# tomer196/GaUDI

Hardware: AMD Instinct MI355X
Metric: guided molecules/sec (1000-step) (higher is better)
Workload: dtype f32

## Files before the change

gaudi_amd/csrc/gaudi_hip.hip:

```cpp
#include <hip/hip_runtime.h>

#include <algorithm>
#include <climits>
#include <queue>
#include <cmath>
#include <cstdio>
#include <cstdlib>
#include <chrono>
#include <cstring>
#include <map>
#include <mutex>
#include <string>
#include <vector>

#include "../../include/gaudi_hip.h"
#include "kernel_table.h"

using namespace gaudi;

struct DevBuf {
  void* p = nullptr;
  size_t cap = 0;
  hipError_t reserve(size_t bytes) {
    if (bytes <= cap) return hipSuccess;
// ... 80 lines not shown
  struct VtCall {
    const gaudi_target_spec* spec = nullptr;
    int K = 0, Btot = 0, b0 = 0;
    float* trace = nullptr;
  }* vt = nullptr;
  PinBuf p_pred, p_dpred;
  PinBuf p_z, p_dz;
  DevBuf d_dz;
  hipEvent_t cb_event = nullptr;
  int steps_per_launch = 25;
  int variant = 8;
  LaunchPlan plan;
  bool split = true;
  bool no_fr = false;
  bool no_n1 = false;
  std::string last_key;
  std::vector<std::string> key_log;
  bool wide_full = true;
  bool gn8_pq = true;
  bool gn8 = true;
  bool force_gn8 = false;
  bool pack = true;
  int pairs_cap = -1;
  int pairs = 1;
  int num_cus = 256;
  bool pred_rounds = true;
  bool pack_now = false;
  bool force_mr = false;
  bool force_gn = false;
  bool fix_noise = false;
// ... 537 lines not shown
      for (int k = 0; k < ns; ++k)
        if (sl[k].live && sl[k].j == j) idx[n_out++] = (uint16_t)k;
    }
    off[N] = (uint16_t)n_out;
  }
  M.order.resize(B);
  for (int b = 0; b < B; ++b) M.order[b] = b;
  std::stable_sort(M.order.begin(), M.order.end(), [&](int a, int c) {
    return M.ntiles[a] != M.ntiles[c] ? M.ntiles[a] > M.ntiles[c] : total[a] > total[c];
  });
  return GAUDI_OK;
}

KernelTable* gaudi::g_kernel_tables;

static kernel_fn find_kernel(const KernelKey& k) {
  for (const KernelTable* t = g_kernel_tables; t; t = t->next)
    for (int i = 0; i < t->n; ++i)
      if (t->entries[i].key == k) return t->entries[i].fn;
  return nullptr;
}
static std::string key_name(const KernelKey& k) {
  char buf[160];
  snprintf(buf, sizeof buf, "waves=%d SP=%d MR=%d GN=%d FR=%d PG=%d N1=%d EF=%d HPE=%d HPP=%d VT=%d", k.waves, k.sp, (int)k.mr, k.gn,
           (int)k.fr, (int)k.pg, (int)k.n1, k.ef, k.hpe, k.hpp, (int)k.vt);
  return buf;
}
static std::string duplicate_kernel_key() {
  std::vector<KernelKey> seen;
  for (const KernelTable* t = g_kernel_tables; t; t = t->next)
    for (int i = 0; i < t->n; ++i) {
      if (std::find(seen.begin(), seen.end(), t->entries[i].key) != seen.end()) return key_name(t->entries[i].key);
      seen.push_back(t->entries[i].key);
    }
  return "";
// ... 172 lines not shown
    }
  }
#else
  if (h->prof) {
    KParams PC = P;
    HIPCHECK(h, h->d_clock.reserve(sizeof(unsigned long long) * 4));
    PC.clock_out = h->d_clock.as<unsigned long long>();
    hipLaunchKernelGGL(fn, dim3(P.B), dim3(v8 ? w8::kThreads : kThreads), lds, h->stream, PC);
  } else {
    hipLaunchKernelGGL(fn, dim3(P.B), dim3(v8 ? w8::kThreads : kThreads), lds, h->stream, P);
  }
#endif
  HIPCHECK(h, hipGetLastError());
  h->last_key = key_name(key);
  if (std::find(h->key_log.begin(), h->key_log.end(), h->last_key) == h->key_log.end()) h->key_log.push_back(h->last_key);
  if (h->prof) {
    HIPCHECK(h, h->prof_log.end(h->stream, ev));
    h->prof_steps += steps;
  }
  return GAUDI_OK;
}

struct Pack {
  int G = 0;
  int NG = 0;
  std::vector<float> umask, uemask;
  std::vector<uint8_t> align;
  std::vector<int32_t> rowmap;
  std::vector<int32_t> compmol;
  std::vector<int32_t> ncomp;
// ... 264 lines not shown
  P.NR = N;
  P.EW = M.S;
  P.node_mask = h->d_mask.as<float>();
  P.order = h->d_order.as<int>();
  P.edges = h->d_edges.as<uint32_t>();
  P.emask = h->d_emask.as<float>();
  P.npairs = h->d_npairs.as<int>();
  P.seginfo = h->d_seg.as<uint32_t>();
  P.ncols = h->d_ncols.as<int>();
  P.soff = h->d_soff.as<uint16_t>();
  P.sidx = h->d_sidx.as<uint16_t>();
  P.rowmap = packed ? h->d_rowmap.as<int32_t>() : nullptr;
  P.compmol = packed ? h->d_compmol.as<int32_t>() : nullptr;
  P.ncomp = packed ? h->d_ncomp.as<int32_t>() : nullptr;
  P.hk_off = 0;
  int hk = 0;
  if (h->keep_h && GAUDI_NODE_F16 && acc.mode >= 1 && nodes == kResident) {
    const size_t floats = lds_bytes8(hpe, hpp, n_slots, Dz, M.S, acc.pubx, acc.mode) / sizeof(float);
    const size_t at = (floats + 3) & ~(size_t)3;
    const size_t need = (size_t)w8::nh_keep_floats(std::max(hpe, hpp), n_slots);
    if ((at + need) * sizeof(float) + 1024 <= 160 * 1024) {
      P.hk_off = (int)at;
      hk = (int)need;
    }
  }
  if (pg_run) {
    const size_t stride = ((size_t)n_slots * (hpp + 4) + 63) / 64 * 64;
    HIPCHECK(h, h->d_gnode.reserve(sizeof(float) * (stride * (size_t)B + 256)));
    P.gnode = h->d_gnode.as<float>();
    P.gnode_stride = (long long)stride;
  }
  if (gn8) {
    const size_t stride = (gnode_floats8(hpe, hpp, N) + 63) / 64 * 64;
    HIPCHECK(h, h->d_gnode.reserve(sizeof(float) * (stride * (size_t)B + 256)));
    P.gnode = h->d_gnode.as<float>();
    P.gnode_stride = (long long)stride;
  }
  plan.waves = 8;
  plan.ring = acc.mode;
  plan.mr = mr_run;
// ... 122 lines not shown
  if (const char* v = getenv("GAUDI_PACK")) h->pack = atoi(v) != 0;
  if (const char* v = getenv("GAUDI_GN8_PACK")) h->gn8_pack = atoi(v) != 0;
  if (const char* v = getenv("GAUDI_GN8_PQ")) h->gn8_pq = atoi(v) != 0;
  if (const char* v = getenv("GAUDI_WIDE_FULL")) h->wide_full = atoi(v) != 0;
  if (const char* v = getenv("GAUDI_KEEP_H")) h->keep_h = atoi(v) != 0;
  if (const char* v = getenv("GAUDI_FAMILY_SPLIT")) h->family_split = atoi(v) != 0;
  if (const char* v = getenv("GAUDI_PAIRS")) h->pairs = atoi(v);
  if (const char* v = getenv("GAUDI_PAIRS_CAP")) h->pairs_cap = atoi(v);
  {
    int cus = 0;
    if (hipDeviceGetAttribute(&cus, hipDeviceAttributeMultiprocessorCount, device) == hipSuccess && cus > 0) h->num_cus = cus;
  }
  if (const char* v = getenv("GAUDI_PRED_ROUNDS")) h->pred_rounds = atoi(v) != 0;
  h->no_fr = getenv("GAUDI_NO_FR") != nullptr;
  h->no_n1 = getenv("GAUDI_NO_N1") != nullptr;
  h->plan.waves = h->variant;
  if (hipSetDevice(device) != hipSuccess || hipStreamCreateWithFlags(&h->stream, hipStreamNonBlocking) != hipSuccess) {
    delete h;
    return GAUDI_E_HIP;
  }
  *out = h;
  return GAUDI_OK;
}

void gaudi_destroy(gaudi_handle* h) {
  if (!h) return;
  (void)hipSetDevice(h->device);
  if (h->stream) (void)hipStreamSynchronize(h->stream);
  h->prof_log.reset(true);
  h->stab_log.reset(true);
// ... 1373 lines not shown
```

gaudi_amd/csrc/kern8s1_fused_192_208.hip:

```cpp
#include "kernel_table.h"

namespace {
using namespace gaudi;
using V = V8T<1, false, 0, false, false, true>;
const KernelEntry kEntries[] = {
    entry<V, 192, 208>(),
};
KernelTable kTable(kEntries);
}
```

gaudi_amd/csrc/kernel_table.h:

```cpp
#pragma once
#include "sampler_kernel.h"

namespace gaudi {

typedef void (*kernel_fn)(const KParams);

struct KernelKey {
  int waves;
  int sp;
  bool mr;
  int gn;
  bool fr, pg;
  bool n1;
  int ef;
  int hpe, hpp;
  bool vt;
};
inline bool operator==(const KernelKey& a, const KernelKey& b) {
  return a.waves == b.waves && a.sp == b.sp && a.mr == b.mr && a.gn == b.gn && a.fr == b.fr && a.pg == b.pg && a.n1 == b.n1 && a.ef == b.ef &&
         a.hpe == b.hpe && a.hpp == b.hpp && a.vt == b.vt;
}

struct KernelEntry {
  KernelKey key;
  kernel_fn fn;
};
template <class V, int HPE, int HPP, bool VT = false>
constexpr KernelEntry entry() {
  KernelEntry e{};
  e.key.waves = V::kWaveCount;
  e.key.sp = V::kSplit;
  e.key.mr = V::kMR;
  e.key.gn = V::kGN;
  e.key.fr = V::kFR;
  e.key.pg = V::kPG;
  e.key.n1 = V::kN1;
  e.key.ef = V::kEF;
  e.key.hpe = HPE;
  e.key.hpp = HPP;
  e.key.vt = VT;
  e.fn = &sampler_kernel_v<V, HPE, HPP, VT>;
  return e;
}

struct KernelTable {
  const KernelEntry* entries;
  int n;
  KernelTable* next;
  template <int N>
  explicit KernelTable(const KernelEntry (&e)[N]);
};
extern KernelTable* g_kernel_tables;
template <int N>
KernelTable::KernelTable(const KernelEntry (&e)[N]) : entries(e), n(N), next(g_kernel_tables) {
  g_kernel_tables = this;
}
// ... 3 lines not shown
```

gaudi_amd/csrc/sampler_kernel.h:

```cpp
#pragma once
#include "edm_device.h"
#include "pred_device.h"
#include "w8_edm.h"
#include "w8_pred.h"

#ifndef GAUDI_STATIC_PRIO
#define GAUDI_STATIC_PRIO 0
#endif

namespace gaudi {

enum Mode { MODE_PHI = 0, MODE_SAMPLE = 1, MODE_PRED_FWD = 2, MODE_PRED_GRAD = 3, MODE_GUIDE = 4, MODE_NLL = 5 };

struct KParams {
  int mode, B, N, F, EW;
  int NR;
  int do_init, do_decode, guided;
  int s_hi, s_lo, T;
  const float* node_mask;
  const int* order;
  const uint32_t* edges;
  const float* emask;
  const int* npairs;
  const uint32_t* seginfo;
// ... 28 lines not shown
  float* stash;
  long long stash_stride;
  float readout_div;
  const float* alpha_sigma;
  float* zt_out;
  int split;
  float* chain_out;
  int keep_frames;
  unsigned long long* stamps;
  float* gnode;
  long long gnode_stride;
  const int32_t* rowmap;
  const int32_t* compmol;
  const int32_t* ncomp;
  unsigned long long* clock_out;
  int hk_off;
  const struct VtDev* vt;
};
struct VtDev {
  const float* par;
  float* trace;
  int top;
  int B;
};
__device__ __forceinline__ const float* vt_row(const VtDev* vt, int b, int K) { return vt->par + (size_t)b * target_row_floats(K); }
__device__ __forceinline__ float* vt_trace_row(const VtDev* vt, int b, int K, int srow) {
  float* const t = vt->trace;
  return t != nullptr ? t + ((size_t)(vt->top - srow) * vt->B + b) * (K + 2) : nullptr;
}
constexpr int kMaxComp = 4;
// ... 1 lines not shown
__host__ __device__ inline int common_floats(int N, int D, int EW) {
  return 3 * align16(N * D) + align16(N) + 16 + align16(N) + 16 + 2 * kWaves * EW + align16(N);
}
__host__ __device__ inline int common_floats8(int N, int D, int S) {
  return 3 * align16(N * D) + align16(N) + 16 + align16(N) + 16 + 2 * S + align16(N) + align16((N + 1 + S + 1) / 2);
}
__device__ __forceinline__ int row_of(int w) { return w & 0x0fffffff; }
__device__ __forceinline__ int comp_of(int w) { return (w >> 28) & 7; }

template <bool GN, int EF = 2>
struct V4T {
  static constexpr int kThreads = gaudi::kThreads;
  static constexpr bool kGlobalNodes = GN;
  static constexpr int kWaveCount = 4, kSplit = 0, kGN = GN ? 1 : 0, kEF = EF;
  static constexpr bool kMR = false, kFR = false, kPG = false, kN1 = false;
  using Graph = gaudi::MolGraph;
  template <int HP> using EdmSmem = gaudi::NetSmem<HP, GN, EF>;
  __device__ __forceinline__ static void set_rows(Graph&, const int*, int, int) {}
  __host__ __device__ static int graph_floats(int N, int EW) { return 2 * gaudi::kWaves * EW + align16(N); }
  __device__ __forceinline__ static float* load_graph(const KParams& P, int b, float* base, const float* sMask, Graph& mg, int tid, int wave) {
    const int N = P.N, EW = P.EW;
    uint32_t* sEdge = (uint32_t*)base; base += gaudi::kWaves * EW;
    float* sEm = base; base += gaudi::kWaves * EW;
    uint32_t* sSeg = (uint32_t*)base; base += align16(N);
    for (int i = tid; i < N; i += kThreads) sSeg[i] = P.seginfo[b * N + i];
    for (int i = tid; i < gaudi::kWaves * EW; i += kThreads) {
      sEdge[i] = P.edges[(size_t)b * gaudi::kWaves * EW + i];
      sEm[i] = P.emask[(size_t)b * gaudi::kWaves * EW + i];
    }
    mg.N = N; mg.D = 3 + P.F; mg.EW = EW;
// ... 134 lines not shown
}
#ifndef GAUDI_STAMPS
template <int HP, int SP, int GN = 0, int FL = 0>
__device__ __attribute__((noinline)) void edm8_call(EdmDev W_, Graph8Args ga_, float t_val_, float* gnode_ = nullptr) {
  extern __shared__ __attribute__((aligned(16))) float smem[];
  const EdmDev W = uni(W_);
  const Graph8Args ga = uni(ga_);
  const float t_val = uni(t_val_);
  const Lds8 L = carve_lds8(smem, ga.N, ga.D, ga.S);
  const w8::MolGraph mg = graph8(L, ga);
  w8::NetSmem<HP, SP, GN> sm;
  sm.carve(L.net, ga.N, ga.S, GN ? uni(gnode_) : nullptr);
  sm.hk = ga.hk ? smem + ga.hk : nullptr;
  w8::edm_forward<HP, SP, GN, FL>(W, mg, sm, L.sZ, L.sEps, L.sMean, t_val, (int)threadIdx.x);
}
template <int HP, int SP, bool MR, int GN = 0, int FL = 0, bool PG = false>
__device__ __attribute__((noinline)) void pred_fwd8_call(PredDev W_, Graph8Args ga_, float t_val_, float* stash_, float readout_div_,
                                                         float* gnode_ = nullptr) {
  extern __shared__ __attribute__((aligned(16))) float smem[];
  const PredDev W = uni(W_);
  const Graph8Args ga = uni(ga_);
  const Lds8 L = carve_lds8(smem, ga.N, ga.D, ga.S);
  const w8::MolGraph mg = graph8(L, ga);
  w8::PredSmem<HP, SP, GN, PG> sm;
  sm.carve(L.net, ga.N, ga.S, ga.pubx, (GN || PG) ? uni(gnode_) : nullptr);
  sm.hk = ga.hk ? smem + ga.hk : nullptr;
  w8::pred_forward<HP, SP, MR, GN, FL>(W, mg, sm, L.sZ, uni(t_val_), uni(stash_), uni(readout_div_), (int)threadIdx.x);
}
template <int HP, int SP, bool MR, int GN = 0, int FL = 0, bool PG = false>
__device__ __attribute__((noinline)) void pred_bwd8_call(PredDev W_, Graph8Args ga_, float* stash_, float readout_div_, int resume_,
                                                         float* gnode_ = nullptr) {
  extern __shared__ __attribute__((aligned(16))) float smem[];
  const PredDev W = uni(W_);
  const Graph8Args ga = uni(ga_);
  const Lds8 L = carve_lds8(smem, ga.N, ga.D, ga.S);
  const w8::MolGraph mg = graph8(L, ga);
  w8::PredSmem<HP, SP, GN, PG> sm;
  sm.carve(L.net, ga.N, ga.S, ga.pubx, (GN || PG) ? uni(gnode_) : nullptr);
  w8::pred_backward<HP, SP, MR, GN, FL>(W, mg, sm, uni(stash_), L.sEps , uni(readout_div_), ga.pub_ch, (int)threadIdx.x,
                        uni(resume_) ? L.sZ : nullptr);
}
#endif

template <int SP, bool MR = false, int GN = 0, bool FR = false, bool PG = false, bool N1 = false>
struct V8T {
  static_assert(!N1 || (!MR && GN == 0 && !FR && !PG), "N1 is a form of the plain resident kernel");
  static constexpr int kFL = N1 ? w8::kNodeOneTile : (MR || GN != 0 || FR) ? w8::kNodeFresh : w8::kNodePlain;
  static constexpr int kThreads = w8::kThreads;
  static constexpr int kSplit = SP;
  static constexpr int kWaveCount = 8, kGN = GN, kEF = 2;
  static constexpr bool kMR = MR, kFR = FR, kPG = PG, kN1 = N1;
  using Graph = w8::MolGraph;
  __host__ __device__ static int graph_floats(int N, int S) { return 2 * S + align16(N) + align16((N + 1 + S + 1) / 2); }
  __device__ __forceinline__ static float* load_graph(const KParams& P, int b, float* base, const float* sMask, Graph& mg, int tid, int wave) {
    (void)wave;
    const int N = P.N, S = P.EW;
    uint32_t* sEdge = (uint32_t*)base; base += S;
    float* sEm = base; base += S;
    uint32_t* sSeg = (uint32_t*)base; base += align16(N);
    uint16_t* sOff = (uint16_t*)base;
    uint16_t* sIdx = sOff + (N + 1);
    base += align16((N + 1 + S + 1) / 2);
    for (int i = tid; i < N; i += kThreads) sSeg[i] = P.seginfo[b * N + i];
    for (int i = tid; i < N + 1; i += kThreads) sOff[i] = P.soff[(size_t)b * (N + 1) + i];
    for (int i = tid; i < S; i += kThreads) {
      sEdge[i] = P.edges[(size_t)b * S + i];
      sEm[i] = P.emask[(size_t)b * S + i];
      sIdx[i] = P.sidx[(size_t)b * S + i];
    }
    mg.N = N; mg.D = 3 + P.F; mg.S = S;
    mg.NC = P.ncols[b];
    mg.ntiles = P.npairs[b];
    mg.rounds = (mg.ntiles + w8::kWaves - 1) / w8::kWaves;
    mg.pubx = P.pubx;
    mg.pub_ch = P.pub_ch;
    mg.hk = P.hk_off;
    mg.mask = sMask; mg.edge = sEdge; mg.em = sEm; mg.seg = sSeg; mg.soff = sOff; mg.sidx = sIdx;
    return base;
  }
  __device__ __forceinline__ static void set_rows(Graph& mg, const int* row, int ncomp, int NR) { mg.row = row; mg.ncomp = ncomp; mg.NR = NR; }
  __device__ __forceinline__ static Graph8Args gargs(const Graph& mg) {
    return Graph8Args{mg.N, mg.D, mg.S, mg.NC, mg.ntiles, mg.pubx, mg.pub_ch, mg.hk};
  }
  static constexpr bool kGlobalNodes = GN != 0 || PG;
  template <int HP>
  __device__ __forceinline__ static void edm(const EdmDev& W, const Graph& mg, float* net, const float* sZ, float* sEps,
                                             float* sMean, float t_val, int tid STAMP_DECL, float* gnode) {
#ifdef GAUDI_STAMPS
    w8::NetSmem<HP, SP, GN> sm;
    sm.carve(net, mg.N, mg.S, GN ? uni(gnode) : nullptr);
    sm.hk = w8::lds_at(mg.hk);
// ... 6 lines not shown
  template <int HP>
  __device__ __forceinline__ static void guide(const PredDev& W, const Graph& mg, float* net, float* sZ, float* sGrad, float* sTmp,
                                               float* sMean, float t_val, float sigma, const float* target_w, float scale,
                                               float* pred_out, float readout_div, float* stash, int tid STAMP_DECL, int phase,
                                               const float* dpred_ext, float* gnode, const float* dz_ext, const VtDev* vt,
                                               int b, int srow) {
#ifdef GAUDI_STAMPS
    (void)vt; (void)b; (void)srow;
    (void)dz_ext;
    w8::guidance_update<HP, SP, MR, GN, PG>(W, mg, net, sZ, sGrad, sTmp, sMean, t_val, sigma, target_w, scale, pred_out, readout_div, stash,
                                            mg.pubx, mg.pub_ch, tid STAMP_ARGS, phase, dpred_ext, (GN || PG) ? uni(gnode) : nullptr);
#else
    (void)sTmp;
    w8::PredSmem<HP, SP, GN, PG> sm;
    sm.carve(net, mg.N, mg.S, mg.pubx, gnode);
    if (phase != 2) pred_fwd8_call<HP, SP, MR, GN, kFL, PG>(W, gargs(mg), t_val, stash, readout_div, gnode);
    if (vt != nullptr) vt_seed8(vt, b, srow, W.K, (int)(sm.pred - lds_base()));
    else w8::guidance_seed(W, sm, target_w, scale, pred_out, tid, phase, dpred_ext);
    if (phase == 1) return;
    pred_bwd8_call<HP, SP, MR, GN, kFL, PG>(W, gargs(mg), stash, readout_div, phase == 2 ? 1 : 0, gnode);
    if (dz_ext != nullptr) {
      for (int e = tid; e < mg.N * mg.D; e += kThreads) sGrad[e] += dz_ext[e];
      __syncthreads();
    }
    if (vt != nullptr) vt_norm8(vt, b, srow, W.K, mg.N * mg.D, (int)(sGrad - lds_base()));
    w8::guidance_apply(mg, sZ, sGrad, sMean, sigma, tid);
    if (vt != nullptr) vt_clip8(vt, b, srow, W.K, (int)(sMean - lds_base()));
#endif
  }
  template <int HP>
  __device__ __forceinline__ static void pred_entry(const PredDev& W, const Graph& mg, float* net, float* sZ, float* sGrad,
// ... 373 lines not shown
```

gaudi_amd/csrc/w8_common.h:

```cpp
#pragma once
#include <type_traits>

#include "device_common.h"

namespace gaudi {
namespace w8 {

constexpr int kWaves = 8;
constexpr int kThreads = 512;

template <int SH>
__device__ __forceinline__ float row_shr(float v) {
  return __builtin_bit_cast(float, __builtin_amdgcn_update_dpp(0, __builtin_bit_cast(int, v), 0x110 + SH, 0xF, 0xF, true));
}

template <int N, class F>
__device__ __forceinline__ void static_for_n(F f) {
  if constexpr (N > 0) {
    static_for_n<N - 1>(f);
    f(std::integral_constant<int, N - 1>{});
  }
}

struct RunMask {
// ... 451 lines not shown
  for (int u = wave; u < units; u += kWaves)
    __builtin_amdgcn_global_load_lds((const __attribute__((address_space(1))) void*)(g + u * 256 + lane * 4),
                                     (__attribute__((address_space(3))) void*)(lds + u * 256), 16, 0, 0);
}
__device__ __forceinline__ void stage_wait() {
  asm volatile("s_waitcnt vmcnt(0)" ::: "memory");
  __syncthreads();
}
__host__ __device__ __forceinline__ constexpr int stage_stride(int floats) { return (floats + 255) & ~255; }

struct MolGraph {
  int N, D, S;
  int NC;
  int ntiles, rounds;
  int pubx, pub_ch;
  int hk = 0;
  const float* mask;
  const uint32_t* edge;
  const float* em;
  const uint32_t* seg;
  const uint16_t* soff;
  const uint16_t* sidx;
  const int* row;
  int ncomp;
  int NR;
};
__device__ __forceinline__ float* lds_at(int off) {
  extern __shared__ __attribute__((aligned(16))) float gaudi_lds_alias[];
  return off ? gaudi_lds_alias + off : nullptr;
}
// ... 5 lines not shown
```

gaudi_amd/csrc/w8_nodes_f16.h:

```cpp
#pragma once
#include "w8_split.h"

namespace gaudi {
namespace w8 {


constexpr float kLoScale = 2048.f;
#ifndef GAUDI_NODE_ABLATE
#define GAUDI_NODE_ABLATE 0
#endif
constexpr int kAblateH = GAUDI_NODE_ABLATE;
#ifndef GAUDI_NODE_STAMPS
#define GAUDI_NODE_STAMPS 0
#endif
#ifndef GAUDI_NODE_PRIO
#define GAUDI_NODE_PRIO 1
#endif
struct NodeStampH {
  unsigned long long sum[8], last;
  __device__ __forceinline__ void start() { last = __builtin_amdgcn_s_memtime(); }
  __device__ __forceinline__ void mark(int i) {
    const unsigned long long t = __builtin_amdgcn_s_memtime();
    sum[i] += t - last;
    last = t;
// ... 178 lines not shown
constexpr int kNodePlain = 0;
constexpr int kNodeFresh = 1;
constexpr int kNodeOneTile = 2;
constexpr int kTailRuntime = 0;
constexpr int kTailOne = 1;

struct NodeCtxH {
  float winv;
  float* split_a;
  float* split_b;
  bool ktail;
  float* scales;
  float* scales_b = nullptr;
};

template <int HP, int EPI, bool TWO, int MAXNT, int PIN = kAheadOne, int POUT = kAheadOne, int FL = kNodePlain, int TAIL = kTailRuntime,
          int NU = 0, class XB = const float*>
__device__ __forceinline__ void node_gemm_h(const WBuf& wh, int Wa, const float* sXa, bool do_split_a, int Wb, const XB& sXb,
                                            const float* sBias, float* sY, const float* sRes, const float* sMask, int N, int wave,
                                            int lane, const NodeCtxH& cx, NodePFH<HP>& pf, int nextW = -1, float* gPre = nullptr,
                                            uint32_t* sMaxOut = nullptr ,
                                            NodeStampH* ns = nullptr) {
  (void)ns;
  using G = NodeGeoH<HP>;
  constexpr int T = G::T, LD = HP + 4, NTW = NU > 0 ? NU : G::NTW, nc = G::nc, D = G::D;
  constexpr int kIn = PIN < D ? PIN : D, kOut = POUT < D ? POUT : D;
  constexpr int kLate = nc < D ? 0 : (GAUDI_NODE_LATE < kOut ? GAUDI_NODE_LATE : kOut);
  constexpr int TQ = TAIL == kTailOne ? 1 : 4;
  const bool ktail = TAIL == kTailOne ? true : cx.ktail;
  constexpr bool kFresh = FL == kNodeFresh;
  const int c = lane & 15, g = lane >> 4;
  const int nt = (MAXNT < 2 || N <= 16) ? 1 : (MAXNT < 3 || N <= 32) ? 2 : 3;
  const bool seq = TWO && cx.split_b == cx.split_a;
  const SplitBufH sa{cx.split_a, nt, cx.scales}, sb{cx.split_b, nt, cx.scales_b != nullptr ? cx.scales_b : cx.scales + kScaleFloatsH};
  const int bpos = nh_bpos(c, g);
  const TileLanesH<HP> tl(wave, lane);
  const TileLanesH<HP> tl_next(wave, lane, nextW >= 0);
  const int Wn = nextW >= 0 ? nextW : Wa;
// ... 22 lines not shown
    if (TWO && !seq) split_rows_h<HP>(sb, sXb, N, wave, ls);
    NSTAMP(1);
    if (do_split_a || (TWO && !seq)) lds_barrier();
    NSTAMP(2);
  }

  f4 acc0[MAXNT][NTW], acc1[MAXNT][NTW], y[MAXNT][NTW];
#pragma unroll
  for (int j = 0; j < MAXNT; ++j)
#pragma unroll
    for (int u = 0; u < NTW; ++u) {
      const int t = wave + kWaves * u < T ? wave + kWaves * u : 0;
      acc0[j][u] = splat(0.f);
      acc1[j][u] = splat(0.f);
      y[j][u] = sBias != nullptr ? *(const f4*)(sBias + 16 * t + 4 * g) : splat(0.f);
    }
  struct BH {
    u4 h, l;
  };
  auto bld = [&](const SplitBufH& s_, int i, int j) {
    const float* q = s_.chunk(i) + bpos + j * 512;
    return BH{*(const u4*)q, *(const u4*)(q + 256)};
  };
  auto mm = [&](const NodeSetH<G::NTW>& s, const BH& b, int j) {
    if (kAblateH & 2) {
      asm volatile("" ::"v"(s.p[0][0]), "v"(s.p[0][1]), "v"(s.p[NTW - 1][0]), "v"(s.p[NTW - 1][1]), "v"(b.h), "v"(b.l));
      return;
    }
#pragma unroll
    for (int u = 0; u < NTW; ++u) acc1[j][u] = mfma_h(s.p[u][0], b.l, acc1[j][u]);
// ... 129 lines not shown
            }
            if (EPI == EPI_MUL_DSILU) {
              const f4 r = *(const f4*)(sRes + nd * LD + 16 * t + 4 * ge);
              yy = yy * dsilu4v(r);
            }
            if (EPI == EPI_ACCUM) yy = *(const f4*)(sRes + nd * LD + 16 * t + 4 * ge) + yy;
          }
          *(f4*)dst = yy;
        }
      }
    }
  });
  NSTAMP(6);
}

#ifndef GAUDI_NODE_F16
#define GAUDI_NODE_F16 1
#endif
template <int SP>
struct NodeMath {
  static constexpr bool kF16 = SP != 0 && GAUDI_NODE_F16 != 0;
};
template <int HP, bool NH>
struct NodePFSel {
  using type = NodePF<HP>;
};
template <int HP>
struct NodePFSel<HP, true> {
  using type = NodePFH<HP>;
};
// ... 47 lines not shown
```

gaudi_amd/csrc/w8_pred.h:

```cpp
#pragma once
#include "pred_device.h"
#include "w8_edm.h"

namespace gaudi {
namespace w8 {

template <int HP, int SP = 0, int GN = 0, bool PG = false>
struct PredSmem {
  static_assert(!(PG && GN != 0), "PG is a variant of the resident kernels");
  static_assert(!GN || SP != 0, "global node buffers: split edge GEMMs only (the fp32 form's publish buffer starts in b0 / b1)");
  static constexpr bool kGlobalNodes = GN != 0;
  float *b2, *b3, *b4;
  float *b0, *b1;
  float* ring;
  float* pub;
  float *x, *x0, *dx;
  uint32_t *pmax, *qmax;
  float* hsc;
  f4* geo;
  float *d0, *trans, *dd0;
  float* pred;
  float* vec;
  float* hk = nullptr;
  __host__ __device__ static int floats(int N, int S, int pubx) {
    return EdgeRing<HP, SP>::kFloats + (GN ? gn_lds_buffers(GN) : PG ? 4 : 5) * N * (HP + 4) + pubx + 12 * N + 2 * align4(N) + 96 + S * 10 + 32 + 10 * HP;
  }
  __device__ __forceinline__ float* publish() const { return GN ? ring : b0; }
  __device__ void carve(float* base, int N, int S, int pubx, float* gnode = nullptr) {
    constexpr int LD = HP + 4;
    if (SP == 0) { ring = base; base += EdgeRing<HP, SP>::kFloats; }
    if (GN || PG) gnode = assume_global(gnode);
    float*& nb = GN ? gnode : base;
    if (GN == 2) { b2 = base; base += N * LD; } else { b2 = nb; nb += N * LD; }
    b3 = nb; nb += N * LD;
    if (PG) { b4 = gnode; gnode += N * LD; } else { b4 = nb; nb += N * LD; }
    b0 = nb; nb += N * LD;
    if (GN == 2) { b1 = base; base += N * LD; } else { b1 = nb; nb += N * LD; }
    if (SP != 0) { ring = base; base += EdgeRing<HP, SP>::kFloats; }
// ... 13 lines not shown
  }
};

__host__ __device__ inline long long pred_stash_floats8(int N, int HP, int L, int S) {
  return pred_stash_node_floats(N, HP, L) + (long long)L * S * HP * 2 + 2LL * L * S + (S > 16 * kWaves ? (long long)S * HP : 0);
}
__device__ __forceinline__ size_t edge_stash_off8(int l, int tile, int arr, int S, int HP) {
  return (((size_t)l * (S / 16) + tile) * 2 + arr) * (size_t)(16 * HP);
}

__host__ __device__ inline int pub_chunk_tiles(int S, long long avail_floats, int T) {
  int ch = (int)((avail_floats / (S > 0 ? S : 1) - 4) / 16);
  return ch > T ? T : ch;
}

template <int HP, int SP = 0, bool MR = false, int GN = 0, int FL = 0, class SM = PredSmem<HP, SP, GN>>
__device__ __forceinline__ void pred_forward(const PredDev& W, const MolGraph& mg, const SM& sm, const float* sZ,
                                             float t_val, float* stash, float readout_div, int tid STAMP_DECL) {
  constexpr int LD = HP + 4;
  constexpr int T = HP / 16;
  const int wave = __builtin_amdgcn_readfirstlane(tid >> 6), lane = tid & 63, c = lane & 15, g = lane >> 4;
  const int N = mg.N, D = mg.D, F = W.F, F1 = F + 1, K = W.K, S = mg.S;
  PredLayout lay{HP, F1, K, W.L};
  const float* __restrict__ w = W.w;
  const WBuf wb = make_wbuf(W.w, W.w_bytes);
  const WBuf wbe = SP ? make_wbuf(W.ws, W.ws_bytes) : wb;
  const bool tw = W.ktail != 0;
  float *h = sm.b0, *p = sm.b1, *q = sm.b2, *agg = sm.b3, *agg1 = sm.b4;
  float* estash = stash + pred_stash_node_floats(N, HP, W.L);
  float* astash = estash + (size_t)W.L * S * HP * 2;
  float* pstash = astash + (size_t)W.L * S;
// ... 25 lines not shown
  constexpr bool STG = GN && !NH;
  float* const xs0 = sm.ring;
  float* const xs1 = sm.ring + stage_stride(N * LD);
  if constexpr (!RI) er_start<HP>(ring, wbe, lay.layer(0) + 2 * HP * HP, wave, lane);
  typename NodePFSel<HP, NH>::type pf;
  node_prefetch_x<HP, NH, kAheadOne>(pf, wb, wbe, lay.layer(0), mg.NC, wave, lane, tw);
  auto hctx = [&]() {
    if constexpr (NH) {
      if constexpr (RI) return node_ctx_h<HP>(sm.ring, EdgeRing<HP, SP>::kFloats, mg.NC, W.hinv, tw, sm.hsc);
      else return node_ctx_h<HP>(ring.slot(ring.par ^ 1), EdgeRing<HP, SP>::kFloats / 2, mg.NC, W.hinv, tw, sm.hsc);
    } else {
      return NodeCtxH{1.f, nullptr, nullptr, tw, nullptr};
    }
  };
  const bool keep = NH && sm.hk != nullptr;
  constexpr int NV = (PredLayerW::vec_count(HP) + kThreads - 1) / kThreads;
  VecPF<NV> vpf;
  vec_prefetch<NV, kThreads>(vpf, wb, PredLayerW::vec_off(lay.layer(0), HP), PredLayerW::vec_count(HP), tid);

  for (int l = 0; l < W.L; ++l) {
    const bool last = l == W.L - 1;
    const PredLayerW Lw(w, lay.layer(l), HP, sm.vec);
    vec_commit<NV, kThreads>(vpf, sm.vec, PredLayerW::vec_count(HP), tid);
    if constexpr (STG) stage_rows(xs0, h, N * LD, wave, lane);
    for (int idx = tid; idx < N * LD; idx += kThreads) {
      agg[idx] = 0.f;
      agg1[idx] = 0.f;
    }
    if (tid < N) {
      sm.pmax[tid] = 0u;
      sm.qmax[tid] = 0u;
    }
    float* st = stash + (size_t)l * (3 * N * HP + 4 * N);
    for (int idx = tid; idx < N; idx += kThreads) gstore4((f4*)(st + 3 * N * HP) + idx, *(const f4*)(sm.x + 4 * idx));
    compute_geo(sm, mg, 1.0f, tid, false);
    if constexpr (STG) stage_wait();
    else __syncthreads();
    STAMP(ST_STAGE);
    {
      const NodeCtxH cx = keep ? node_ctx_keep<HP>(hctx(), sm.hk, mg.NC) : hctx();
      node_gemm_x<HP, EPI_NONE, false, GN, NH, kAheadOne, kAheadAll, FL>(wb, wbe, Lw.A, h, xs0, true, -1, nullptr, nullptr, Lw.b1, p, nullptr, nullptr, mg.NC, wave,
                                                    lane, tw, cx, pf, Lw.Bm, nullptr, sm.pmax);
      node_gemm_x<HP, EPI_NONE, false, GN, NH, kAheadAll, kAheadOne, FL>(wb, wbe, Lw.Bm, h, xs0, false, -1, nullptr, nullptr, nullptr, q, nullptr, nullptr, mg.NC,
                                                    wave, lane, tw, cx, pf, Lw.Wn1h, nullptr, sm.qmax);
    }
    STAMP(ST_NODE);
    __syncthreads();
    STAMP(ST_BARRIER);
    if constexpr (RI) er_start<HP>(ring, wbe, Lw.W2, wave, lane);
    for (int idx = tid; idx < N * (HP / 4); idx += kThreads) {
      const int n = idx / (HP / 4), f = 4 * (idx % (HP / 4));
      nstash_store((f4*)st + idx, *(const f4*)(p + n * LD + f));
      nstash_store((f4*)(st + N * HP) + idx, *(const f4*)(q + n * LD + f));
    }
    STAMP(ST_STASH);
    int rd = 0;
    {
    pred_fwd_round:
      const bool more = MR && rd + 1 < mg.rounds;
      const TileCols tc = load_tile(mg, MR ? rd : 0, wave, c);
      const f4 gg = sm.geo[tc.slot];
      f4 acc[T];
      const float d0f = sm.d0[tc.slot];
      const float ub = __builtin_bit_cast(float, sm.pmax[tc.i]) + __builtin_bit_cast(float, sm.qmax[tc.j]) + sm.vec[9 * HP + 1] * gg[0] +
                       sm.vec[9 * HP + 2] * fabsf(d0f);
      er_gemm_pq<HP>(acc, ring, wbe, Lw.W2, last ? (more ? Lw.W2 : -1) : Lw.Wc1, Lw.b2, Lw.cr, Lw.cd, p + tc.i * LD + 4 * g,
                       q + tc.j * LD + 4 * g, gg[0], d0f, ub, tc.active, wave, lane STAMP_ARGS);
      STAMP(ST_EDGE);
      const int tile = tc.slot >> 4;
      if (tc.active) {
        {
// ... 47 lines not shown
    STAMP(ST_BARRIER);
    constexpr bool SUM = NH && GN == 0;
    if constexpr (!SUM) {
      if constexpr (STG) stage_rows(xs0, h, N * LD, wave, lane);
      for (int idx = tid; idx < N * (HP / 4); idx += kThreads) {
        const int n = idx / (HP / 4), f = 4 * (idx % (HP / 4));
        if constexpr (STG)
          *(f4*)(xs1 + n * LD + f) = *(const f4*)(agg + n * LD + f) + *(const f4*)(agg1 + n * LD + f);
        else
          *(f4*)(agg + n * LD + f) = *(const f4*)(agg + n * LD + f) + *(const f4*)(agg1 + n * LD + f);
      }
      if constexpr (STG) stage_wait();
      else __syncthreads();
    }
    STAMP(ST_MISC);
    node_gemm_x<HP, EPI_SILU, true, GN, NH, kAheadOne, kAheadOne, FL, SUM ? 1 : 0>(
        wb, wbe, Lw.Wn1h, h, xs0, !keep, Lw.Wn1a, agg, xs1, Lw.bn1, p, nullptr, nullptr, mg.NC, wave, lane, tw,
        keep ? node_ctx_keep<HP>(hctx(), sm.hk, mg.NC) : hctx(), pf, Lw.Wn2, st + 2 * N * HP , nullptr, agg1);
    STAMP(ST_NODE);
    __syncthreads();
    STAMP(ST_BARRIER);
    vec_prefetch<NV, kThreads>(vpf, wb, PredLayerW::vec_off(lay.layer(l + 1 < W.L ? l + 1 : l), HP), PredLayerW::vec_count(HP), tid);
    if constexpr (STG) {
      stage_rows(xs0, p, N * LD, wave, lane);
      stage_wait();
    }
    node_gemm_x<HP, EPI_RESIDUAL_MASK, false, GN, NH, kAheadOne, kAheadOne, FL>(wb, wbe, Lw.Wn2, p, xs0, true, -1, nullptr, nullptr, Lw.bn2, h, h, mg.mask, mg.NC, wave,
                                                     lane, tw, hctx(), pf, l + 1 < W.L ? lay.layer(l + 1) : -1);
    if (!last) coord_update(sm, mg, 1.0f, tid);
    STAMP(ST_NODE);
// ... 457 lines not shown
```

gaudi_amd/csrc/w8_split.h:

```cpp
#pragma once
#include "w8_common.h"
#ifndef GAUDI_EDGE_PRIO
#define GAUDI_EDGE_PRIO 0
#endif


namespace gaudi {
namespace w8 {

typedef _Float16 h8 __attribute__((ext_vector_type(8)));
typedef _Float16 h2 __attribute__((ext_vector_type(2)));
typedef __attribute__((ext_vector_type(2))) float f2;
typedef __attribute__((ext_vector_type(4))) uint32_t u4;
typedef __attribute__((ext_vector_type(2))) uint32_t u2;
constexpr int kPieces = 2;

template <int N, class F>
__device__ __forceinline__ void static_for(F f) {
  if constexpr (N > 0) {
    static_for<N - 1>(f);
    f(std::integral_constant<int, N - 1>{});
  }
}

// ... 113 lines not shown
  using G = SplitGeo<HP, MODE>;
  int off, units;
  if (!trip_group(r, W, nextW, tr, off, units)) return false;
  static_assert(G::UT * G::kUnit * 4 <= 4096, "a wave's units must lie within the immediate offset of its first");
  const int first = (unsigned)(wave * units) / kWaves, count = (unsigned)((wave + 1) * units) / kWaves - first;
  dma_units<0, G::UT, G::kUnit * 4>(wb, (off + first * G::kUnit) * 4, lane, slot + first * G::kUnit, count);
  return true;
}
template <int HP, int MODE>
__device__ __forceinline__ void rings_start(RingS<HP, MODE>& r, const WBuf& wb, int W, int wave, int lane) {
  rings_dma(r, wb, r.slot(r.par), W, -1, 0, wave, lane);
}
template <int HP, int MODE>
__device__ __forceinline__ void rings_stage(RingS<HP, MODE>& r, const WBuf& wb, int W, int nextW, int tr, int wave, int lane) {
  rings_dma(r, wb, r.slot(r.par ^ 1), W, nextW, tr + 1, wave, lane);
}

__device__ __forceinline__ void trip_barrier() {
  asm volatile("s_waitcnt vmcnt(0)" ::: "memory");
  __syncthreads();
}
template <int HP, int MODE>
__device__ __forceinline__ void trip_open(RingS<HP, MODE>& r, int lane) {
  (void)r;
  (void)lane;
  trip_barrier();
}
template <int HP, int MODE>
__device__ __forceinline__ void trip_close(RingS<HP, MODE>& r, int lane) {
  (void)lane;
// ... 258 lines not shown
```

Baseline: 221.7.

## Overlap node GEMM h-part on a side wave during edge-ring trips

Adds a 'side job' variant of the N1 predictor kernel. The last wave computes the h-dependent half of the first node GEMM (Wn1h·h plus bias) into a dedicated LDS region while the other waves run the edge ring trips. The later node GEMM then starts from these precomputed rows and only applies Wn1a to the aggregated messages. This takes serial node-GEMM work off the critical path in exchange for extra LDS, a custom barrier/DMA split that drops one wave from the edge stage, and more host planning logic.

```diff
diff --git a/gaudi_amd/csrc/gaudi_hip.hip b/gaudi_amd/csrc/gaudi_hip.hip
--- a/gaudi_amd/csrc/gaudi_hip.hip
+++ b/gaudi_amd/csrc/gaudi_hip.hip
@@ -118,6 +118,7 @@
   bool split = true;
   bool no_fr = false;
   bool no_n1 = false;
+  bool no_side = false;
   std::string last_key;
   std::vector<std::string> key_log;
   bool wide_full = true;
@@ -685,11 +686,15 @@
 
 KernelTable* gaudi::g_kernel_tables;
 
-static kernel_fn find_kernel(const KernelKey& k) {
+static const KernelEntry* find_entry(const KernelKey& k) {
   for (const KernelTable* t = g_kernel_tables; t; t = t->next)
     for (int i = 0; i < t->n; ++i)
-      if (t->entries[i].key == k) return t->entries[i].fn;
+      if (t->entries[i].key == k) return &t->entries[i];
   return nullptr;
+}
+static kernel_fn find_kernel(const KernelKey& k) {
+  const KernelEntry* e = find_entry(k);
+  return e ? e->fn : nullptr;
 }
 static std::string key_name(const KernelKey& k) {
   char buf[160];
@@ -892,6 +897,8 @@
   HIPCHECK(h, hipGetLastError());
   h->last_key = key_name(key);
   if (std::find(h->key_log.begin(), h->key_log.end(), h->last_key) == h->key_log.end()) h->key_log.push_back(h->last_key);
+  if (const KernelEntry* e = find_entry(key); e && (e->side & 1) && P.side_off != 0) h->last_key += " SD=" + std::to_string(e->side);
+  if (getenv("GAUDI_DEBUG_PLAN")) fprintf(stderr, "[launch] %s\n", h->last_key.c_str());
   if (h->prof) {
     HIPCHECK(h, h->prof_log.end(h->stream, ev));
     h->prof_steps += steps;
@@ -1186,16 +1193,30 @@
   P.compmol = packed ? h->d_compmol.as<int32_t>() : nullptr;
   P.ncomp = packed ? h->d_ncomp.as<int32_t>() : nullptr;
   P.hk_off = 0;
+  P.side_off = 0;
   int hk = 0;
+  bool side_run = false;
   if (h->keep_h && GAUDI_NODE_F16 && acc.mode >= 1 && nodes == kResident) {
     const size_t floats = lds_bytes8(hpe, hpp, n_slots, Dz, M.S, acc.pubx, acc.mode) / sizeof(float);
     const size_t at = (floats + 3) & ~(size_t)3;
     const size_t need = (size_t)w8::nh_keep_floats(std::max(hpe, hpp), n_slots);
-    if ((at + need) * sizeof(float) + 1024 <= 160 * 1024) {
+    KernelKey kn = key8(hpe, hpp, 1, false);
+    kn.n1 = true;
+    const KernelEntry* const en = find_entry(kn);
+    const bool side_want = !h->no_side && n1_run && hpe && hpp && !mr_run && en != nullptr && (en->side & 1) &&
+                           *std::max_element(M.ntiles.begin(), M.ntiles.begin() + B) <= w8::kWaves - 1;
+    const size_t side = (size_t)n_slots * (hpp + 4);
+    if (side_want && (at + side + need) * sizeof(float) + 1024 <= 160 * 1024) {
+      P.side_off = (int)at;
+      P.hk_off = (int)(at + side);
+      hk = (int)need;
+      side_run = true;
+    } else if ((at + need) * sizeof(float) + 1024 <= 160 * 1024) {
       P.hk_off = (int)at;
       hk = (int)need;
     }
   }
+  if (getenv("GAUDI_DEBUG_PLAN")) fprintf(stderr, "[plan] side=%d side_off=%d hk_off=%d hk=%d\n", (int)side_run, P.side_off, P.hk_off, hk);
   if (pg_run) {
     const size_t stride = ((size_t)n_slots * (hpp + 4) + 63) / 64 * 64;
     HIPCHECK(h, h->d_gnode.reserve(sizeof(float) * (stride * (size_t)B + 256)));
@@ -1348,6 +1369,7 @@
   if (const char* v = getenv("GAUDI_PRED_ROUNDS")) h->pred_rounds = atoi(v) != 0;
   h->no_fr = getenv("GAUDI_NO_FR") != nullptr;
   h->no_n1 = getenv("GAUDI_NO_N1") != nullptr;
+  h->no_side = getenv("GAUDI_NO_SIDE") != nullptr;
   h->plan.waves = h->variant;
   if (hipSetDevice(device) != hipSuccess || hipStreamCreateWithFlags(&h->stream, hipStreamNonBlocking) != hipSuccess) {
     delete h;
diff --git a/gaudi_amd/csrc/kern8s1_fused_192_208.hip b/gaudi_amd/csrc/kern8s1_fused_192_208.hip
--- a/gaudi_amd/csrc/kern8s1_fused_192_208.hip
+++ b/gaudi_amd/csrc/kern8s1_fused_192_208.hip
@@ -1,8 +1,12 @@
 #include "kernel_table.h"
+
+#ifndef GAUDI_SIDE_STAGES
+#define GAUDI_SIDE_STAGES 1
+#endif
 
 namespace {
 using namespace gaudi;
-using V = V8T<1, false, 0, false, false, true>;
+using V = V8T<1, false, 0, false, false, true, GAUDI_SIDE_STAGES>;
 const KernelEntry kEntries[] = {
     entry<V, 192, 208>(),
 };
diff --git a/gaudi_amd/csrc/kernel_table.h b/gaudi_amd/csrc/kernel_table.h
--- a/gaudi_amd/csrc/kernel_table.h
+++ b/gaudi_amd/csrc/kernel_table.h
@@ -24,6 +24,7 @@
 struct KernelEntry {
   KernelKey key;
   kernel_fn fn;
+  int side;
 };
 template <class V, int HPE, int HPP, bool VT = false>
 constexpr KernelEntry entry() {
@@ -40,6 +41,7 @@
   e.key.hpp = HPP;
   e.key.vt = VT;
   e.fn = &sampler_kernel_v<V, HPE, HPP, VT>;
+  e.side = HPP != 0 ? V::kSD : 0;
   return e;
 }
 
diff --git a/gaudi_amd/csrc/sampler_kernel.h b/gaudi_amd/csrc/sampler_kernel.h
--- a/gaudi_amd/csrc/sampler_kernel.h
+++ b/gaudi_amd/csrc/sampler_kernel.h
@@ -66,6 +66,7 @@
   const int32_t* compmol;
   const int32_t* ncomp;
   unsigned long long* clock_out;
+  int side_off;
   int hk_off;
   const struct VtDev* vt;
 };
@@ -97,6 +98,7 @@
   static constexpr bool kGlobalNodes = GN;
   static constexpr int kWaveCount = 4, kSplit = 0, kGN = GN ? 1 : 0, kEF = EF;
   static constexpr bool kMR = false, kFR = false, kPG = false, kN1 = false;
+  static constexpr int kSD = 0;
   using Graph = gaudi::MolGraph;
   template <int HP> using EdmSmem = gaudi::NetSmem<HP, GN, EF>;
   __device__ __forceinline__ static void set_rows(Graph&, const int*, int, int) {}
@@ -261,9 +263,9 @@
   sm.hk = ga.hk ? smem + ga.hk : nullptr;
   w8::edm_forward<HP, SP, GN, FL>(W, mg, sm, L.sZ, L.sEps, L.sMean, t_val, (int)threadIdx.x);
 }
-template <int HP, int SP, bool MR, int GN = 0, int FL = 0, bool PG = false>
+template <int HP, int SP, bool MR, int GN = 0, int FL = 0, bool PG = false, int SD = 0>
 __device__ __attribute__((noinline)) void pred_fwd8_call(PredDev W_, Graph8Args ga_, float t_val_, float* stash_, float readout_div_,
-                                                         float* gnode_ = nullptr) {
+                                                         float* gnode_ = nullptr, int side_ = 0) {
   extern __shared__ __attribute__((aligned(16))) float smem[];
   const PredDev W = uni(W_);
   const Graph8Args ga = uni(ga_);
@@ -272,7 +274,8 @@
   w8::PredSmem<HP, SP, GN, PG> sm;
   sm.carve(L.net, ga.N, ga.S, ga.pubx, (GN || PG) ? uni(gnode_) : nullptr);
   sm.hk = ga.hk ? smem + ga.hk : nullptr;
-  w8::pred_forward<HP, SP, MR, GN, FL>(W, mg, sm, L.sZ, uni(t_val_), uni(stash_), uni(readout_div_), (int)threadIdx.x);
+  if constexpr (SD != 0) sm.side = w8::lds_at(uni(side_));
+  w8::pred_forward<HP, SP, MR, GN, FL, SD>(W, mg, sm, L.sZ, uni(t_val_), uni(stash_), uni(readout_div_), (int)threadIdx.x);
 }
 template <int HP, int SP, bool MR, int GN = 0, int FL = 0, bool PG = false>
 __device__ __attribute__((noinline)) void pred_bwd8_call(PredDev W_, Graph8Args ga_, float* stash_, float readout_div_, int resume_,
@@ -289,9 +292,11 @@
 }
 #endif
 
-template <int SP, bool MR = false, int GN = 0, bool FR = false, bool PG = false, bool N1 = false>
+template <int SP, bool MR = false, int GN = 0, bool FR = false, bool PG = false, bool N1 = false, int SD = 0>
 struct V8T {
   static_assert(!N1 || (!MR && GN == 0 && !FR && !PG), "N1 is a form of the plain resident kernel");
+  static_assert(SD == 0 || N1, "the side job is a form of the N1 kernel");
+  static constexpr int kSD = SD;
   static constexpr int kFL = N1 ? w8::kNodeOneTile : (MR || GN != 0 || FR) ? w8::kNodeFresh : w8::kNodePlain;
   static constexpr int kThreads = w8::kThreads;
   static constexpr int kSplit = SP;
@@ -322,6 +327,7 @@
     mg.pubx = P.pubx;
     mg.pub_ch = P.pub_ch;
     mg.hk = P.hk_off;
+    mg.side = P.side_off;
     mg.mask = sMask; mg.edge = sEdge; mg.em = sEm; mg.seg = sSeg; mg.soff = sOff; mg.sidx = sIdx;
     return base;
   }
@@ -358,7 +364,7 @@
     (void)sTmp;
     w8::PredSmem<HP, SP, GN, PG> sm;
     sm.carve(net, mg.N, mg.S, mg.pubx, gnode);
-    if (phase != 2) pred_fwd8_call<HP, SP, MR, GN, kFL, PG>(W, gargs(mg), t_val, stash, readout_div, gnode);
+    if (phase != 2) pred_fwd8_call<HP, SP, MR, GN, kFL, PG, SD>(W, gargs(mg), t_val, stash, readout_div, gnode, SD != 0 ? mg.side : 0);
     if (vt != nullptr) vt_seed8(vt, b, srow, W.K, (int)(sm.pred - lds_base()));
     else w8::guidance_seed(W, sm, target_w, scale, pred_out, tid, phase, dpred_ext);
     if (phase == 1) return;
diff --git a/gaudi_amd/csrc/w8_common.h b/gaudi_amd/csrc/w8_common.h
--- a/gaudi_amd/csrc/w8_common.h
+++ b/gaudi_amd/csrc/w8_common.h
@@ -489,6 +489,7 @@
   int NC;
   int ntiles, rounds;
   int pubx, pub_ch;
+  int side = 0;
   int hk = 0;
   const float* mask;
   const uint32_t* edge;
diff --git a/gaudi_amd/csrc/w8_nodes_f16.h b/gaudi_amd/csrc/w8_nodes_f16.h
--- a/gaudi_amd/csrc/w8_nodes_f16.h
+++ b/gaudi_amd/csrc/w8_nodes_f16.h
@@ -216,14 +216,19 @@
   float* scales_b = nullptr;
 };
 
+struct YInitBias {};
+struct YInitRows {
+  const float* y;
+};
 template <int HP, int EPI, bool TWO, int MAXNT, int PIN = kAheadOne, int POUT = kAheadOne, int FL = kNodePlain, int TAIL = kTailRuntime,
-          int NU = 0, class XB = const float*>
-__device__ __forceinline__ void node_gemm_h(const WBuf& wh, int Wa, const float* sXa, bool do_split_a, int Wb, const XB& sXb,
+          int NU = 0, class XB = const float*, class XA = const float*, class YI = YInitBias>
+__device__ __forceinline__ void node_gemm_h(const WBuf& wh, int Wa, const XA& sXa, bool do_split_a, int Wb, const XB& sXb,
                                             const float* sBias, float* sY, const float* sRes, const float* sMask, int N, int wave,
                                             int lane, const NodeCtxH& cx, NodePFH<HP>& pf, int nextW = -1, float* gPre = nullptr,
                                             uint32_t* sMaxOut = nullptr ,
-                                            NodeStampH* ns = nullptr) {
+                                            NodeStampH* ns = nullptr, const YI& yinit = YI{}) {
   (void)ns;
+  (void)yinit;
   using G = NodeGeoH<HP>;
   constexpr int T = G::T, LD = HP + 4, NTW = NU > 0 ? NU : G::NTW, nc = G::nc, D = G::D;
   constexpr int kIn = PIN < D ? PIN : D, kOut = POUT < D ? POUT : D;
@@ -276,6 +281,8 @@
       acc0[j][u] = splat(0.f);
       acc1[j][u] = splat(0.f);
       y[j][u] = sBias != nullptr ? *(const f4*)(sBias + 16 * t + 4 * g) : splat(0.f);
+      if constexpr (std::is_same<YI, YInitRows>::value)
+        y[j][u] = j * 16 + c < N ? *(const f4*)(yinit.y + (j * 16 + c) * LD + 16 * t + 4 * g) : splat(0.f);
     }
   struct BH {
     u4 h, l;
@@ -435,6 +442,107 @@
   NSTAMP(6);
 }
 
+template <int HP>
+struct SideGeoH {
+  static constexpr int T = HP / 16, nc = nh_chunks(HP), TG = 7;
+  static constexpr int NG = (T + TG - 1) / TG;
+  static constexpr int kSteps = NG * nc;
+  static constexpr bool odd = nh_odd(HP);
+  static_assert(nc >= 1, "at least one fp16 chunk");
+  __host__ __device__ static constexpr int tiles(int gq) { return (gq + 1) * TG <= T ? TG : T - gq * TG; }
+  __host__ __device__ static constexpr int loads(int s) {
+    return (s < 0 || s >= kSteps) ? 0 : tiles(s / nc) * (2 + ((odd && s % nc == nc - 1) ? 1 : 0));
+  }
+};
+template <int HP>
+struct SideJobH {
+  using G = SideGeoH<HP>;
+  u4 w[G::TG][2];
+  float tw[G::TG];
+  f4 acc0[G::TG], acc1[G::TG];
+};
+struct SideArgsH {
+  WBuf wh;
+  int W;
+  const float* bias;
+  SplitBufH x;
+  float winv;
+  float* out;
+  int N;
+};
+template <int HP, int S>
+__device__ __forceinline__ void side_issue(SideJobH<HP>& job, const SideArgsH& a, int lane) {
+  using G = SideGeoH<HP>;
+  if constexpr (S < G::kSteps) {
+    constexpr int gq = S / G::nc, m = S % G::nc;
+    static_for<G::tiles(gq)>([&](auto u_tag) {
+      constexpr int u = decltype(u_tag)::value, t = gq * G::TG + u;
+      const int so = (2 * a.W + m * nh_chunk_floats(HP)) * 4 + t * 2048;
+      job.w[u][0] = __builtin_bit_cast(u4, __builtin_amdgcn_raw_buffer_load_b128(a.wh.r, lane * 16, so, GAUDI_NODE_LOAD_AUX));
+      job.w[u][1] = __builtin_bit_cast(u4, __builtin_amdgcn_raw_buffer_load_b128(a.wh.r, lane * 16 + 1024, so, GAUDI_NODE_LOAD_AUX));
+    });
+    if constexpr (G::odd && m == G::nc - 1)
+      static_for<G::tiles(gq)>([&](auto u_tag) {
+        constexpr int u = decltype(u_tag)::value, t = gq * G::TG + u;
+        job.tw[u] = __builtin_bit_cast(float, __builtin_amdgcn_raw_buffer_load_b32(a.wh.r, lane * 4, (2 * a.W + nh_tail_off(HP) + t * 256) * 4, 0));
+      });
+  }
+}
+template <int HP, int S>
+__device__ __forceinline__ void side_compute(SideJobH<HP>& job, const SideArgsH& a, int lane) {
+  using G = SideGeoH<HP>;
+  if constexpr (S < G::kSteps) {
+    constexpr int gq = S / G::nc, m = S % G::nc, NT = G::tiles(gq), LD = HP + 4;
+    const int c = lane & 15, g = lane >> 4;
+    if constexpr (m == 0)
+      static_for<NT>([&](auto u_tag) {
+        constexpr int u = decltype(u_tag)::value;
+        job.acc0[u] = splat(0.f);
+        job.acc1[u] = splat(0.f);
+      });
+    const float* q = a.x.chunk(m) + nh_bpos(c, g);
+    const u4 bh = *(const u4*)q, bl = *(const u4*)(q + 256);
+    static_for<NT>([&](auto u_tag) { constexpr int u = decltype(u_tag)::value; job.acc1[u] = mfma_h(job.w[u][0], bl, job.acc1[u]); });
+    static_for<NT>([&](auto u_tag) { constexpr int u = decltype(u_tag)::value; job.acc0[u] = mfma_h(job.w[u][0], bh, job.acc0[u]); });
+    static_for<NT>([&](auto u_tag) { constexpr int u = decltype(u_tag)::value; job.acc1[u] = mfma_h(job.w[u][1], bh, job.acc1[u]); });
+    if constexpr (m == G::nc - 1) {
+      const float xt = G::odd ? a.x.tail(HP)[g * 16 + c] : 0.f;
+      const float sc = a.x.scale(HP)[c] * a.winv;
+      static_for<NT>([&](auto u_tag) {
+        constexpr int u = decltype(u_tag)::value, t = gq * G::TG + u;
+        f4 y = a.bias != nullptr ? *(const f4*)(a.bias + 16 * t + 4 * g) : splat(0.f);
+        if constexpr (G::odd) y = mfma1(job.tw[u], xt, y);
+        y = y + (job.acc0[u] + job.acc1[u] * (1.0f / kLoScale)) * sc;
+        if (c < a.N) *(f4*)(a.out + c * LD + 16 * t + 4 * g) = y;
+      });
+    }
+  }
+}
+template <int HP, int S>
+__device__ __forceinline__ void side_rest(SideJobH<HP>& job, const SideArgsH& a, int lane) {
+  if constexpr (S < SideGeoH<HP>::kSteps) {
+    side_compute<HP, S>(job, a, lane);
+    __builtin_amdgcn_sched_barrier(0);
+    side_issue<HP, S + 1>(job, a, lane);
+    side_rest<HP, S + 1>(job, a, lane);
+  }
+}
+template <int HP, int MODE, int S0>
+__device__ __forceinline__ void side_trips(RingS<HP, MODE>& ring, const WBuf& wb, int W, int nextW, int lane, SideJobH<HP>& job,
+                                           const SideArgsH& a) {
+  static_for<side_trip_count<HP, MODE>()>([&](auto tr_tag) {
+    constexpr int tr = decltype(tr_tag)::value, s = S0 + tr;
+    side_barrier<SideGeoH<HP>::loads(s)>();
+    RingsStageSide<HP, MODE, tr>::run(ring, wb, W, nextW, lane);
+    __builtin_amdgcn_sched_barrier(0);
+    side_compute<HP, s>(job, a, lane);
+    __builtin_amdgcn_sched_barrier(0);
+    side_issue<HP, s + 1>(job, a, lane);
+    __builtin_amdgcn_sched_barrier(0);
+    ring.par ^= 1;
+  });
+}
+
 #ifndef GAUDI_NODE_F16
 #define GAUDI_NODE_F16 1
 #endif
diff --git a/gaudi_amd/csrc/w8_pred.h b/gaudi_amd/csrc/w8_pred.h
--- a/gaudi_amd/csrc/w8_pred.h
+++ b/gaudi_amd/csrc/w8_pred.h
@@ -22,6 +22,7 @@
   float* pred;
   float* vec;
   float* hk = nullptr;
+  float* side = nullptr;
   __host__ __device__ static int floats(int N, int S, int pubx) {
     return EdgeRing<HP, SP>::kFloats + (GN ? gn_lds_buffers(GN) : PG ? 4 : 5) * N * (HP + 4) + pubx + 12 * N + 2 * align4(N) + 96 + S * 10 + 32 + 10 * HP;
   }
@@ -65,7 +66,7 @@
   return ch > T ? T : ch;
 }
 
-template <int HP, int SP = 0, bool MR = false, int GN = 0, int FL = 0, class SM = PredSmem<HP, SP, GN>>
+template <int HP, int SP = 0, bool MR = false, int GN = 0, int FL = 0, int SD = 0, class SM = PredSmem<HP, SP, GN>>
 __device__ __forceinline__ void pred_forward(const PredDev& W, const MolGraph& mg, const SM& sm, const float* sZ,
                                              float t_val, float* stash, float readout_div, int tid STAMP_DECL) {
   constexpr int LD = HP + 4;
@@ -121,6 +122,8 @@
     }
   };
   const bool keep = NH && sm.hk != nullptr;
+  constexpr bool kSideA = (SD & 1) != 0;
+  static_assert(!kSideA || (NH && !MR && GN == 0 && !RI && FL == kNodeOneTile), "the side job is a form of the resident N1 kernel");
   constexpr int NV = (PredLayerW::vec_count(HP) + kThreads - 1) / kThreads;
   VecPF<NV> vpf;
   vec_prefetch<NV, kThreads>(vpf, wb, PredLayerW::vec_off(lay.layer(0), HP), PredLayerW::vec_count(HP), tid);
@@ -128,6 +131,7 @@
   for (int l = 0; l < W.L; ++l) {
     const bool last = l == W.L - 1;
     const PredLayerW Lw(w, lay.layer(l), HP, sm.vec);
+    const bool side_l = kSideA && sm.side != nullptr && !last && (tw || !SplitGeo<HP, SP == 0 ? 1 : SP>::kTailOK);
     vec_commit<NV, kThreads>(vpf, sm.vec, PredLayerW::vec_count(HP), tid);
     if constexpr (STG) stage_rows(xs0, h, N * LD, wave, lane);
     for (int idx = tid; idx < N * LD; idx += kThreads) {
@@ -149,7 +153,7 @@
       node_gemm_x<HP, EPI_NONE, false, GN, NH, kAheadOne, kAheadAll, FL>(wb, wbe, Lw.A, h, xs0, true, -1, nullptr, nullptr, Lw.b1, p, nullptr, nullptr, mg.NC, wave,
                                                     lane, tw, cx, pf, Lw.Bm, nullptr, sm.pmax);
       node_gemm_x<HP, EPI_NONE, false, GN, NH, kAheadAll, kAheadOne, FL>(wb, wbe, Lw.Bm, h, xs0, false, -1, nullptr, nullptr, nullptr, q, nullptr, nullptr, mg.NC,
-                                                    wave, lane, tw, cx, pf, Lw.Wn1h, nullptr, sm.qmax);
+                                                    wave, lane, tw, cx, pf, side_l ? Lw.Wn1a : Lw.Wn1h, nullptr, sm.qmax);
     }
     STAMP(ST_NODE);
     __syncthreads();
@@ -162,6 +166,17 @@
     }
     STAMP(ST_STASH);
     int rd = 0;
+    if (side_l && wave == kWaves - 1) {
+      if constexpr (kSideA) {
+        constexpr int n = side_trip_count<HP, SP>();
+        SideJobH<HP> job;
+        const SideArgsH sa{wbe, Lw.Wn1h, Lw.bn1, SplitBufH{sm.hk + kScaleFloatsH, 1, sm.hk}, W.hinv, sm.side, mg.NC};
+        side_issue<HP, 0>(job, sa, lane);
+        side_trips<HP, SP, 0>(ring, wbe, split_off(Lw.W2), split_off(Lw.Wc1), lane, job, sa);
+        side_trips<HP, SP, n>(ring, wbe, split_off(Lw.Wc1), split_off(lay.layer(l + 1) + 2 * HP * HP), lane, job, sa);
+        side_rest<HP, 2 * n>(job, sa, lane);
+      }
+    } else
     {
     pred_fwd_round:
       const bool more = MR && rd + 1 < mg.rounds;
@@ -239,6 +254,13 @@
       else __syncthreads();
     }
     STAMP(ST_MISC);
+    if constexpr (kSideA) {
+      if (side_l)
+        node_gemm_h<HP, EPI_SILU, false, 1, kAheadOne, kAheadOne, FL, nh_odd(HP) ? kTailOne : kTailRuntime>(
+            wbe, Lw.Wn1a, RowsSum<false>{agg, agg1, 1.f}, true, -1, (const float*)nullptr, nullptr, p, nullptr, nullptr, mg.NC, wave, lane,
+            hctx(), pf, Lw.Wn2, st + 2 * N * HP , nullptr, nullptr, YInitRows{sm.side});
+    }
+    if (!side_l)
     node_gemm_x<HP, EPI_SILU, true, GN, NH, kAheadOne, kAheadOne, FL, SUM ? 1 : 0>(
         wb, wbe, Lw.Wn1h, h, xs0, !keep, Lw.Wn1a, agg, xs1, Lw.bn1, p, nullptr, nullptr, mg.NC, wave, lane, tw,
         keep ? node_ctx_keep<HP>(hctx(), sm.hk, mg.NC) : hctx(), pf, Lw.Wn2, st + 2 * N * HP , nullptr, agg1);
diff --git a/gaudi_amd/csrc/w8_split.h b/gaudi_amd/csrc/w8_split.h
--- a/gaudi_amd/csrc/w8_split.h
+++ b/gaudi_amd/csrc/w8_split.h
@@ -151,6 +151,38 @@
 template <int HP, int MODE>
 __device__ __forceinline__ void rings_stage(RingS<HP, MODE>& r, const WBuf& wb, int W, int nextW, int tr, int wave, int lane) {
   rings_dma(r, wb, r.slot(r.par ^ 1), W, nextW, tr + 1, wave, lane);
+}
+
+template <int HP, int MODE>
+__host__ __device__ constexpr int side_trip_count() {
+  return SplitGeo<HP, MODE>::kTailOK ? SplitGeo<HP, MODE>::kTripsTail : SplitGeo<HP, MODE>::kTrips;
+}
+template <int HP, int MODE, int TR>
+struct RingsStageSide {
+__device__ __forceinline__ static void run(const RingS<HP, MODE>& r, const WBuf& wb, int W, int nextW, int lane) {
+  using G = SplitGeo<HP, MODE>;
+  constexpr int n = side_trip_count<HP, MODE>();
+  constexpr bool nxt = TR + 1 >= n;
+  constexpr int t2 = nxt ? TR + 1 - n : TR + 1;
+  constexpr bool tt = G::kTailOK && t2 == n - 1;
+  constexpr int units = tt ? G::T : G::tiles_of(t2 % G::NH) * kPieces;
+  constexpr int rel = tt ? (G::NC - 1) * G::T * kPieces * G::kUnit : ((t2 / G::NH) * G::T + (t2 % G::NH) * G::CH) * kPieces * G::kUnit;
+  constexpr int first = (unsigned)((kWaves - 1) * units) / kWaves, count = units - first;
+  static_assert(count <= G::UT, "the side wave's share of a group");
+  const int vo = lane * 16;
+  const int off = __builtin_amdgcn_readfirstlane(((nxt ? nextW : W) + rel + first * G::kUnit) * 4);
+  float* const l = r.slot(r.par ^ 1) + first * G::kUnit;
+  static_for<count>([&](auto u_tag) {
+    constexpr int U = decltype(u_tag)::value;
+    __builtin_amdgcn_raw_ptr_buffer_load_lds(wb.r, (__attribute__((address_space(3))) void*)l, 16, vo, off, U * G::kUnit * 4, 0);
+  });
+}
+};
+template <int PENDING>
+__device__ __forceinline__ void side_barrier() {
+  asm volatile("s_waitcnt vmcnt(%0) lgkmcnt(0)" ::"n"(PENDING) : "memory");
+  __builtin_amdgcn_s_barrier();
+  asm volatile("" ::: "memory");
 }
 
 __device__ __forceinline__ void trip_barrier() {
```

After: 224.0 (median of 6 runs). +1.0%, better.
